# hartikainen/mujoco_mpc

Hardware: AMD Instinct MI355X
Metric: candidate rollouts/s (horizon x samples) (higher is better)
Workload: dtype f64

## Files before the change

mujoco_mpc_amd/csrc/core.h:

```cpp
#pragma once
#include "dmath.h"
#include "model.h"
#include "linalg.h"
#include "philox.h"

#ifdef MJPC_EMU
static thread_local double *g_emu_lds = nullptr;
static thread_local int g_emu_r = 0;
typedef const KParams *KP;
DEV const KParams *kp_generic(KP k) { return k; }
DEV double *lds_base() { return g_emu_lds; }
DEV int cand_index() { return g_emu_r; }
DEV int uniform_i(int v) { return v; }
#else
extern __shared__ __align__(16) double g_lds[];
typedef const __attribute__((address_space(4))) KParams *KP;
DEV const KParams *kp_generic(KP k) {
  unsigned long long v = (unsigned long long)k;
  unsigned lo = __builtin_amdgcn_readfirstlane((unsigned)v), hi = __builtin_amdgcn_readfirstlane((unsigned)(v >> 32));
  KP u = (KP)(((unsigned long long)hi << 32) | lo);
  return (const KParams *)u;
}
DEV double *lds_base() { return g_lds; }
DEV int cand_index() { return (int)blockIdx.x; }
// ... 211 lines not shown
  }
  PFOR(i, M.nmocap) {
    d_copy3(c.mocap_pos + 3 * i, K->mocap + 7 * i);
    d_copy4(c.mocap_quat + 4 * i, K->mocap + 7 * i + 3);
  }
  PFOR(i, nq) { c.qpos[i] = K->state[i]; R.states[i] = K->state[i]; }
  PFOR(i, nv) { c.qvel[i] = K->state[nq + i]; R.states[nq + i] = K->state[nq + i]; c.qacc_ws[i] = 0; }
  if (M.na) PFOR(i, M.na) { C_ACT(c)[i] = K->state[nq + nv + i]; R.states[nq + nv + i] = K->state[nq + nv + i]; C_ACTDOT(c)[i] = 0; }
  PFOR(e, nv * M.nvp) c.qM[e] = 0;
  if (K->L.Linv - K->L.qH >= nv * M.nvp) PFOR(e, nv * M.nvp) c.qH[e] = 0;
#ifndef MJPC_LEAN_LDS
  PFOR(e, M.nhpair + nv) c.hpair[e] = MI(hpair_i)[e] | (MI(hpair_j)[e] << 8);
#endif
#ifndef MJPC_LEAN_LDS
  PFOR(k, 6 * M.nbody) c.xfrc[k] = 0;
#endif
  PFOR(k, nu) c.ctrl[k] = 0;
  if (LANE == 0) {
    R.times[0] = K->time;
    for (int k = 0; k < 3; k++) { c.xpos[k] = 0; c.xipos[k] = 0; c.subtree_linvel[k] = 0; }
    c.xquat[0] = 1; c.xquat[1] = 0; c.xquat[2] = 0; c.xquat[3] = 0;
    for (int k = 0; k < 9; k++) { c.xmat[k] = (k % 4 == 0) ? 1.0 : 0.0; c.ximat[k] = c.xmat[k]; }
    for (int k = 0; k < 6; k++) { c.cvel[k] = 0; c.cfrc[k] = 0; c.cacc[k] = (k >= 3) ? -M.gravity[k - 3] : 0.0; }
    for (int k = 0; k < MISC_INTS; k++) c.misc[k] = 0;
#if defined(MJPC_PROFILE) && !defined(MJPC_EMU)
    for (int q = 0; q < NPROF; q++) c.prof[q] = 0;
    c.prof[NPROF] = (long long)__builtin_amdgcn_s_memtime();
#endif
  }
  c.time = K->time;
  ctx_close(c);
}

template <int NVT>
DEV_NOINLINE void ph_head(KP Kc, int t, int last) {
  Ctx c; ctx_open(c, Kc);
  const KParams *K = c.K;
  const DevModel &M = *c.M;
  Rows R = out_rows(K);
  int nu = M.nu;
  if (!last) {
    PFOR(k, nu) {
      double a = spline_sample(c.knot_times, c.knot_values, K->P, nu, K->interp, c.time, k);
      a = d_clip(a, MD(actuator_ctrlrange)[2 * k], MD(actuator_ctrlrange)[2 * k + 1]);
      c.ctrl[k] = a; R.actions[t * nu + k] = a;
    }
    SYNC();
    if (bad_values(c.qpos, M.nq)) c.warning |= WARN_BADQPOS;
    if (bad_values(c.qvel, M.nv)) c.warning |= WARN_BADQVEL;
    if (c.warning) { if (LANE == 0) c.misc[10] = 1; ctx_close(c); return; }
    if (K->xfrc_std > 0) {
      double rate = exp(-M.timestep / K->xfrc_rate), scale = K->xfrc_std * sqrt(1 - rate * rate);
      unsigned gi = (unsigned)(K->offset + cand_index());
      int n6 = 6 * M.nbody;
      PFOR(i, n6) c.xfrc[i] = rate * c.xfrc[i] + scale * philox_normal(K->seed, K->stream ^ XFRC_STREAM, gi, (unsigned)(t * n6 + i));
    }
  }
  PROF(c, 0);
  kinematics(c); PROF(c, 1);
#if !MJPC_SIDE_COM
  com_pos(c);
#endif
  PROF(c, 2);
  ctx_close(c);
}
DEV_NOINLINE void ph_constraints(KP Kc, int t) {
  Ctx c; ctx_open(c, Kc);
  collision(c); PROF(c, 4);
  int nsingle, n_nc;
#if MJPC_HELPER
#if MJPC_SIDE_COM
  if (!flag_wait(c.misc + HX_COM, t + 1)) c.warning |= WARN_SYNC;
#endif
  if (!flag_wait(c.misc + 24, t + 1)) c.warning |= WARN_SYNC;
  nsingle = uniform_i(c.misc[25]); n_nc = uniform_i(c.misc[26]);
  c.nsingle = nsingle;
  make_contact_rows(c, n_nc); PROF(c, 5);
  make_impedance(c, n_nc, c.nefc, 1); PROF(c, 7);
#else
  make_noncontact_rows(c, &nsingle, &n_nc);
  c.nsingle = nsingle;
  make_contact_rows(c, n_nc); PROF(c, 5);
  make_impedance(c, 0, c.nefc, 1); PROF(c, 7);
#endif
  ctx_close(c);
}
#if MJPC_HELPER
DEV_NOINLINE void ph_noncontact(KP Kc, int t) {
  Ctx c; ctx_open(c, Kc, 1);
  int nsingle, n_nc;
#if MJPC_SIDE_COM
  if (c.M->neq_connect) { if (!flag_wait(c.misc + HX_COM, t + 1)) c.warning |= WARN_SYNC; }
#endif
  make_noncontact_rows(c, &nsingle, &n_nc);
  if (LANE == 0) { c.misc[25] = nsingle; c.misc[26] = n_nc; }
  flag_set(c.misc + 24, t + 1);
// ... 44 lines not shown
DEV_SOLVE_PHASE void ph_solve(KP Kc, int last, int t) {
  Ctx c; ctx_open(c, Kc);
  c.hseq = t * 256;
  solve_constraints<NVT>(c); PROF(c, 8);
#if MJPC_HELPER
  if (MJPC_SOLVER_REG && NVT > 0) { if (c.M->cone == 1) flag_set(c.misc + HX_JOBW, JOBW(++c.hseq, 0, 0)); }
  else {
    if (LANE == 0) c.misc[HX_KIND] = 0;
    flag_set(c.misc + HX_JOB, ++c.hseq);
  }
#endif
  if (!last && !(c.warning & (WARN_CONTACTFULL | WARN_CNSTRFULL)) && bad_values(c.qacc, c.M->nv)) c.warning |= WARN_BADQACC;
  ctx_close(c);
}
template <int NVT>
DEV_NOINLINE void ph_noslip(KP Kc, int last) {
  Ctx c; ctx_open(c, Kc);
  if (!(c.warning & (WARN_CONTACTFULL | WARN_CNSTRFULL | WARN_SYNC | WARN_BADQACC))) {
    noslip_pass<NVT>(c);
    if (!last && bad_values(c.qacc, c.M->nv)) c.warning |= WARN_BADQACC;
  }
  ctx_close(c);
}
#if MJPC_HELPER
template <int NVT>
DEV_NOINLINE void ph_solve_helper(KP Kc, int t) {
  Ctx c; ctx_open(c, Kc, 1);
  int k = WAVE_ID() - 1;
  static_for<0, MJPC_NH>([&](auto Kc_) { constexpr int KK = decltype(Kc_)::value; if (k == KK) solver_helper_loop<NVT, KK>(c, t * 256); });
}
#endif

struct CostOut { double cost; int warning; };
DEV_NOINLINE CostOut ph_residual_cost(KP Kc, int t, int last) {
  Ctx c; ctx_open(c, Kc, 1);
  const KParams *K = c.K;
  const DevModel &M = *c.M;
  const DevTask &T = M.task;
  Rows R = out_rows(K);
  if (last) PFOR(k, M.nu) R.actions[t * M.nu + k] = (K->H > 1) ? c.ctrl[k] : 0.0;
  if (t == 0 && cand_index() == 0 && K->frame) {
    int nb = M.nbody, ns = M.nsite;
    double *f = K->frame;
    PFOR(i, 3 * nb) { f[i] = c.xpos[i]; f[12 * nb + 3 * ns + i] = c.subtree_com[i]; f[15 * nb + 3 * ns + i] = c.subtree_linvel[i]; }
    PFOR(i, 9 * nb) f[3 * nb + i] = c.xmat[i];
    PFOR(i, 3 * ns) f[12 * nb + i] = c.site_xpos[i];
  }
  task_residual(c, c.residual); PROF(c, 9); PROFW(c, 9);
  PFOR(i, R.nr) R.residual[t * R.nr + i] = c.residual[i];
  PFOR(i, T.num_trace) {
    int id = MI(task.trace_objid)[i], ty = MI(task.trace_objtype)[i];
    const double *src = ty == 6 ? c.site_xpos + 3 * id : (ty == 5 ? c.geom_xpos + 3 * id : (ty == 1 ? c.xipos + 3 * id : c.xpos + 3 * id));
    d_copy3(R.trace + t * R.ntr + 3 * i, src);
  }
  CostOut o;
  o.cost = cost_value(c, c.residual);
  if (LANE == 0) R.costs[t] = o.cost;
  o.warning = c.warning;
  PROF(c, 10); PROFW(c, 10);
  ctx_close(c);
  return o;
}

template <int NVT>
DEV void prefactor_body(Ctx &c) {
  const DevModel &M = *c.M;
  {
    int nv = M.nv, nvp = M.nvp;
    double h = M.timestep;
    PFOR(e, nv * nvp) { int i = e / nvp, j = e - i * nvp; c.qL[e] = c.qM[e] + ((i == j) ? h * MD(dof_damping)[i] : 0.0); }
    if (M.nidrv) {
      SYNC();
      if (LANE == 0)
        for (int k = 0; k < M.nidrv; k++) {
          int i = MI(idrv_e)[3 * k], j = MI(idrv_e)[3 * k + 1], a = MI(idrv_e)[3 * k + 2];
          if (a >= 0 && MI(actuator_forcelimited)[a]) {
            double f = c.actuator_force[a];
            if (f <= MD(actuator_forcerange)[2 * a] || f >= MD(actuator_forcerange)[2 * a + 1]) continue;
          }
          double v = h * MD(idrv_c)[k];
          c.qL[i * nvp + j] += v;
          if (i != j) c.qL[j * nvp + i] += v;
        }
      SYNC();
    }
    chol_factor<NVT>(c.qL, c.Linv, c.scr_a, nv, nvp, c.M->tree_ok);
  }
}
template <int NVT>
DEV_NOINLINE void ph_prefactor(KP Kc) {
  Ctx c; ctx_open(c, Kc, 1);
// ... 134 lines not shown
        d_sub3(off, c.xipos + 3 * b, c.subtree_com + 3 * MIH(body_rootid)[b]);
        const double *ci = c.cdof + 6 * i, *cj = c.cdof + 6 * j;
        d_cross(t, ci, off); for (int k = 0; k < 3; k++) { wi[k] = ci[k]; wi[3 + k] = ci[3 + k] + t[k]; }
        d_cross(t, cj, off); for (int k = 0; k < 3; k++) { wj[k] = cj[k]; wj[3 + k] = cj[3 + k] + t[k]; }
        d_mulmattvec3(li, R, wi); d_mulmattvec3(li + 3, R, wi + 3);
        d_mulmattvec3(lj, R, wj); d_mulmattvec3(lj + 3, R, wj + 3);
        for (int k = 0; k < 6; k++) acc += li[k] * dl[k] * lj[k];
      }
      A[i * nvp + j] += h * acc;
    }
    SYNC();
  }
  if (M.int_dense == 2) implicit_rne_columns(c, A, h);
  for (int k = 0; k < nv; k++) {
    SYNC();
    const double piv = A[k * nvp + k];
    PFOR(ii, nv - k - 1) { int i = k + 1 + ii; A[i * nvp + k] = d_div(A[i * nvp + k], piv); }
    SYNC();
    PFOR(e, (nv - k - 1) * (nv - k - 1)) {
      int i = k + 1 + e / (nv - k - 1), j = k + 1 + e % (nv - k - 1);
      A[i * nvp + j] -= A[i * nvp + k] * A[k * nvp + j];
    }
  }
  SYNC();
  double *x = c.Mgrad;
  if (LANE == 0) {
    for (int i = 0; i < nv; i++) { double s = x[i]; for (int j = 0; j < i; j++) s -= A[i * nvp + j] * x[j]; x[i] = s; }
    for (int i = nv - 1; i >= 0; i--) { double s = x[i]; for (int j = i + 1; j < nv; j++) s -= A[i * nvp + j] * x[j]; x[i] = d_div(s, A[i * nvp + i]); }
  }
  SYNC();
}

template <int NVT>
DEV_NOINLINE void ph_integrate(KP Kc, int t) {
  Ctx c; ctx_open(c, Kc);
  const KParams *K = c.K;
  const DevModel &M = *c.M;
  Rows R = out_rows(K);
  int nq = M.nq, nv = M.nv, nvp = M.nvp;
  double h = M.timestep;
  if (M.noslip_iterations <= 0) { PFOR(i, nv) c.qacc_ws[i] = c.qacc[i]; }
  else if (M.any_damping && !M.int_dense) { prefactor_body<NVT>(c); SYNC(); }
  if (M.int_dense) {
    PFOR(i, nv) c.Mgrad[i] = c.qfrc_smooth[i] + c.qfrc_constraint[i];
    SYNC();
    implicit_dense_solve<NVT>(c);
    PFOR(i, nv) c.qvel[i] += h * c.Mgrad[i];
  } else if (M.any_damping) {
    PFOR(i, nv) c.Mgrad[i] = c.qfrc_smooth[i] + c.qfrc_constraint[i];
    chol_solve<NVT>(c.qL, c.Linv, c.Mgrad, nv, nvp, c.M->tree_ok);
    PFOR(i, nv) c.qvel[i] += h * c.Mgrad[i];
  } else {
    PFOR(i, nv) c.qvel[i] += h * c.qacc[i];
  }
  SYNC();
  PFOR(j, M.njnt) {
    int qa = MIH(jnt_qposadr)[j], da = MIH(jnt_dofadr)[j], type = MIH(jnt_type)[j];
    if (type == 0) {
      for (int k = 0; k < 3; k++) c.qpos[qa + k] += h * c.qvel[da + k];
      d_quatintegrate(c.qpos + qa + 3, c.qvel + da + 3, h);
    } else if (type == 1) {
      d_quatintegrate(c.qpos + qa, c.qvel + da, h);
    } else c.qpos[qa] += h * c.qvel[da];
  }
  if (M.na) {
    PFOR(i, M.nu) {
      int dt = MI(actuator_dyntype)[i];
      if (dt) {
        int a = MI(actuator_actadr)[i];
        double act = C_ACT(c)[a], ad = C_ACTDOT(c)[a];
        if (dt == DYN_FILTEREXACT) { double tau = fmax(D_MINVAL, MD(actuator_dynprm)[i]); act += ad * tau * (1 - exp(-h / tau)); }
        else act += h * ad;
        if (MI(actuator_actlimited)[i]) act = d_clip(act, MD(actuator_actrange)[2 * i], MD(actuator_actrange)[2 * i + 1]);
        C_ACT(c)[a] = act;
        R.states[(t + 1) * R.ds + nq + nv + a] = act;
      }
    }
  }
  c.time += h;
  SYNC();
  PFOR(i, nq) R.states[(t + 1) * R.ds + i] = c.qpos[i];
  PFOR(i, nv) R.states[(t + 1) * R.ds + nq + i] = c.qvel[i];
  if (LANE == 0) R.times[t + 1] = c.time;
  PROF(c, 11);
  ctx_close(c);
}

#define CKPT_HEAD 7
DEV_NOINLINE void ph_finish(KP Kc, double total, int failure, int t_fail, double total_before) {
  Ctx c; ctx_open(c, Kc, 1);
  const KParams *K = c.K;
  int r = cand_index(), H = K->H;
  if (K->tier > 0 && K->ckpt) {
    double *ck = K->ckpt + (size_t)r * K->ckpt_stride;
    const DevModel &M = *c.M;
    int resumable = failure && (c.warning & (WARN_CONTACTFULL | WARN_CNSTRFULL)) && !(c.warning & ~(WARN_CONTACTFULL | WARN_CNSTRFULL)) && !(K->xfrc_std > 0);
    if (LANE == 0) {
      ck[0] = resumable ? 1.0 : 0.0; ck[1] = (double)t_fail; ck[2] = c.time; ck[3] = total_before;
      ck[4] = (double)c.misc[5]; ck[5] = (double)c.misc[6]; ck[6] = (double)c.misc[7];
    }
    if (resumable) {
      PFOR(i, M.nq) ck[CKPT_HEAD + i] = c.qpos[i];
      PFOR(i, M.nv) { ck[CKPT_HEAD + M.nq + i] = c.qvel[i]; ck[CKPT_HEAD + M.nq + M.nv + i] = c.qacc_ws[i]; }
      if (M.na) PFOR(i, M.na) ck[CKPT_HEAD + M.nq + 2 * M.nv + i] = C_ACT(c)[i];
    }
  }
  if (LANE == 0) {
    K->returns[r] = failure ? 1.0e6 : total / (H > 1 ? H : 1);
    K->failure[r] = failure ? (c.warning ? c.warning : 1) : 0;
#if defined(MJPC_PROFILE) && !defined(MJPC_EMU)
    if (K->prof) for (int q = 0; q < NPROF; q++) K->prof[(size_t)r * NPROF + q] = c.prof[q];
#endif
    if (K->diag) { K->diag[4 * r] = c.misc[5]; K->diag[4 * r + 1] = c.misc[6]; K->diag[4 * r + 2] = c.misc[7]; K->diag[4 * r + 3] = c.warning; }
  }
}

DEV_NOINLINE void ph_resume(KP Kc) {
// ... 5 lines not shown
  PFOR(i, M.nv) { c.qvel[i] = ck[CKPT_HEAD + M.nq + i]; c.qacc_ws[i] = ck[CKPT_HEAD + M.nq + M.nv + i]; }
  if (M.na) PFOR(i, M.na) C_ACT(c)[i] = ck[CKPT_HEAD + M.nq + 2 * M.nv + i];
  if (LANE == 0) { c.misc[5] = (int)ck[4]; c.misc[6] = (int)ck[5]; c.misc[7] = (int)ck[6]; }
  c.time = ck[2];
  ctx_close(c);
}

template <int NVT>
DEV void rollout(KP Kc) {
  int H = Kc->H;
  const bool r0 = ROLE0, r1 = ROLE1;
  if (r0) ph_init(Kc);
  XBAR();
  const int *misc = (const int *)(lds_base() + Kc->L.ints) + Kc->L.i_misc;
  double total = 0, total_before = 0;
  int failure = 0, t0 = 0, t_fail = 0;
  if (Kc->retry && Kc->ckpt) {
    const double *ck = Kc->ckpt + (size_t)cand_index() * Kc->ckpt_stride;
    if (ck[0] != 0.0) {
      t0 = (int)ck[1]; total = ck[3];
      if (r0) ph_resume(Kc);
      XBAR();
    }
  }
#if defined(MJPC_PROFILE) && !defined(MJPC_EMU)
  long long *rprof = (long long *)(lds_base() + Kc->L.prof);
#define RPROF(i) do { if (LANE == 0 && WAVE_ID() == MJPC_PROFILE_WAVE) PROF_STAMP(rprof, i); } while (0)
#else
#define RPROF(i) ((void)0)
#endif
  for (int t = t0; t < H; t++) {
    int last = (t == H - 1);
    t_fail = t; total_before = total;
    if (r0) ph_head<NVT>(Kc, t, last);
    XBAR(); RPROF(2);
    if (uniform_i(misc[10])) { failure = 1; break; }
    if (r0) ph_constraints(Kc, t);
    if (r1) ph_smooth<NVT>(Kc, t);
#if MJPC_HELPER
    if (ROLEH && WAVE_ID() == 1) ph_inertia<NVT>(Kc, t);
    if (ROLEH && WAVE_ID() == MJPC_WAVES - 2) ph_noncontact(Kc, t);
#endif
    XBAR(); RPROF(3);
    if (r0) { ph_solve<NVT>(Kc, last, t); if (Kc->M.noslip_iterations > 0) ph_noslip<NVT>(Kc, last); }
#if MJPC_HELPER
    if (ROLEH) ph_solve_helper<NVT>(Kc, t);
#endif
    if (r1) {
      CostOut o = ph_residual_cost(Kc, t, last); total += o.cost;
      if (!last) ph_prefactor<NVT>(Kc);
#if MJPC_HELPER
      ph_side_worker<NVT>(Kc, t);
#endif
    }
    XBAR(); RPROF(6);
    if (uniform_i(misc[3]) | uniform_i(misc[11])) { failure = 1; break; }
    if (r0 && !last) ph_integrate<NVT>(Kc, t);
  }
  XBAR();
  if (r1) ph_finish(Kc, total, failure, t_fail, total_before);
}
```

mujoco_mpc_amd/csrc/linalg.h:

```cpp
#pragma once
#include <type_traits>
#include "dmath.h"
#include "model.h"

struct Ctx;

#ifndef MJPC_EMU
DEV double readlane_d(double v, int lane) {
  int lo = __builtin_amdgcn_readlane(__double2loint(v), lane);
  int hi = __builtin_amdgcn_readlane(__double2hiint(v), lane);
  return __hiloint2double(hi, lo);
}
#endif

DEV void chol_factor_lds(double *A, double *Linv, double *tmp, int n, int nvp) {
  for (int j = 0; j < n; j++) {
    SYNC();
    PFOR(ii, n - j) {
      int i = j + ii;
      double s = A[i * nvp + j];
#pragma unroll 4
      for (int k = 0; k < j; k++) s -= A[i * nvp + k] * A[j * nvp + k];
      tmp[i] = s;
    }
    SYNC();
    double t = tmp[j];
    if (t < D_MINVAL) t = D_MINVAL;
    double dj = sqrt(t), inv = 1.0 / dj;
    PFOR(ii, n - j) {
      int i = j + ii;
      A[i * nvp + j] = (i == j) ? dj : tmp[i] * inv;
    }
    if (LANE == 0) Linv[j] = inv;
  }
  SYNC();
}
DEV void chol_solve_lds(const double *L, const double *Linv, double *x, int n, int nvp) {
  for (int i = 0; i < n; i++) {
    SYNC();
    double xi = x[i] * Linv[i];
    SYNC();
    PFOR(kk, n - i - 1) { int k = i + 1 + kk; x[k] -= L[k * nvp + i] * xi; }
    if (LANE == 0) x[i] = xi;
  }
  for (int i = n - 1; i >= 0; i--) {
    SYNC();
    double xi = x[i] * Linv[i];
    SYNC();
    PFOR(k, i) x[k] -= L[i * nvp + k] * xi;
    if (LANE == 0) x[i] = xi;
  }
  SYNC();
}

#ifndef MJPC_EMU
template <int N>
struct LDLRegs { double lo[N], up[N], rinv; };
struct LDLExtra { const double *x[3]; int n; const double *row; };

template <int I, int E, class F>
DEV void static_for(F &&f) {
  if constexpr (I < E) { f(std::integral_constant<int, I>{}); static_for<I + 1, E>(f); }
}
template <int N>
DEV void ldl_load_row(const double *A, int nvp, const LDLExtra *ex, double *a, double &dg) {
  const int i = LANE;
  const bool act = i < N;
  if (ex && ex->row) {
    double d0 = 1.0;
    static_for<0, N>([&](auto jc) { constexpr int j = decltype(jc)::value; a[j] = act ? ex->row[j] : 0.0; d0 = (j == i) ? ex->row[j] : d0; });
    dg = act ? d0 : 1.0;
  } else {
    static_for<0, N>([&](auto jc) { constexpr int j = decltype(jc)::value; a[j] = act ? A[(j <= i) ? i * nvp + j : j * nvp + i] : 0.0; });
    dg = act ? A[i * nvp + i] : 1.0;
  }
  if (ex && ex->n > 0) {
    const int nx = ex->n;
    double t[3][N], td[3];
#pragma unroll
    for (int w = 0; w < 3; w++) {
      const double *X = ex->x[w < nx ? w : 0];
      static_for<0, N>([&](auto jc) { constexpr int j = decltype(jc)::value; t[w][j] = X[(j <= i && act) ? i * nvp + j : (act ? j * nvp + i : 0)]; });
      td[w] = X[act ? i * nvp + i : 0];
      if (w + 1 >= nx) break;
    }
    __builtin_amdgcn_sched_barrier(0);
#pragma unroll
    for (int w = 0; w < 3; w++) {
      if (w >= nx) break;
      static_for<0, N>([&](auto jc) { constexpr int j = decltype(jc)::value; a[j] += act ? t[w][j] : 0.0; });
      dg += act ? td[w] : 0.0;
    }
  }
}
template <int N>
DEV void ldl_factor_regs(const double *A, int nvp, LDLRegs<N> &f, const LDLExtra *ex = nullptr) {
  static_assert(N >= 1 && N <= 64, "one matrix row per lane");
  const int i = LANE;
  const bool act = i < N;
  double a[N];
  double dg;
  ldl_load_row<N>(A, nvp, ex, a, dg);
  static_for<1, N>([&](auto kc) {
// ... 192 lines not shown
```

mujoco_mpc_amd/csrc/solver_reg.h:

```cpp
#pragma once
#ifndef MJPC_EMU
#ifndef LS_PREDICT
#define LS_PREDICT 1
#endif

template <int NVT> struct HLay {
  static constexpr int G0 = 64 / NVT;
  static constexpr int G = G0 < 1 ? 1 : (G0 > NVT ? NVT : G0);
  static constexpr int CB = (NVT + G - 1) / G;
};
DEV int readlane_i(int v, int lane) { return __builtin_amdgcn_readlane(v, lane); }
#define LSR_STRIDE 7
#define LSC_STRIDE 17
#define LS_ROWREC(c) ((c).efc_JA + 64)
#define LS_CONREC(c) ((c).efc_JA + 64 + (c).M->nefcmax * LSR_STRIDE)

template <int NVT>
DEV void hblock_add_rows(const Ctx &c, double *h, unsigned long long mask, int rbase, double wlane, int hi, int j0) {
  constexpr int nvp = NVP_OF(NVT), CB = HLay<NVT>::CB;
  while (mask) {
    int b0 = (int)__builtin_ctzll(mask); mask &= mask - 1;
    int b1 = b0; double sel1 = 0.0;
    if (mask) { b1 = (int)__builtin_ctzll(mask); mask &= mask - 1; sel1 = 1.0; }
    double w0 = readlane_d(wlane, b0), w1 = readlane_d(wlane, b1) * sel1;
// ... 112 lines not shown
#if defined(MJPC_PROFILE) && !defined(MJPC_EMU)
    if (MJPC_PROFILE_WAVE != 0 && WAVE_ID() == MJPC_PROFILE_WAVE) { int na_ = __builtin_popcountll(__builtin_amdgcn_ballot_w64(active)); if (LANE == 0) { c.prof[23] += na_; c.prof[22] += (it0 == p0 * NLANE); } }
#endif
    if constexpr (DIMT > 3) {
#pragma unroll
      for (int k = 3; k < DIMT; k++) { const bool in = k < dim; P[k] = in ? P[k] : 0.0; Q[k] = in ? Q[k] : 0.0; T[k] = in ? T[k] : 0.0; ji[k] = in ? ji[k] : 0.0; }
    }
    double pi = P[0] * ji[0], qi = Q[1] * ji[1];
#pragma unroll
    for (int k = 1; k < DIMT; k++) { pi += P[k] * ji[k]; if (k > 1) qi += Q[k] * ji[k]; }
    double t[DIMT];
    t[0] = P[0] * pi + Q[0] * ji[0];
#pragma unroll
    for (int k = 1; k < DIMT; k++) t[k] = P[k] * pi - Q[k] * qi + (T[k] * T[k]) * ji[k];
    double *prow = part + i * nvp;
    PROFW(c, 16);
    for (int b = 0; __builtin_amdgcn_ballot_w64(active && b <= a) != 0; b += 2) {
      const bool on0 = active && b <= a, on1 = active && b + 1 <= a;
      const int j0 = dofs[on0 ? b : 0], j1 = dofs[on1 ? b + 1 : 0];
      double x0[DIMT], x1[DIMT];
#pragma unroll
      for (int k = 0; k < DIMT; k++) { x0[k] = Jr[(DIMT <= 3 || k < dim ? k : 0) * nvp + j0]; x1[k] = Jr[(DIMT <= 3 || k < dim ? k : 0) * nvp + j1]; }
      __builtin_amdgcn_sched_barrier(0);
      double v0 = t[0] * x0[0], v1 = t[0] * x1[0];
#pragma unroll
      for (int k = 1; k < DIMT; k++) { v0 += t[k] * x0[k]; v1 += t[k] * x1[k]; }
      if (on0) __builtin_amdgcn_ds_atomic_fadd_f64((__attribute__((address_space(3))) double *)(prow + j0), v0);
      if (on1) __builtin_amdgcn_ds_atomic_fadd_f64((__attribute__((address_space(3))) double *)(prow + j1), v1);
    }
  }
}

#if MJPC_HELPER
DEV int jobw_load(const Ctx &c) { return __builtin_amdgcn_readfirstlane(__hip_atomic_load(c.misc + HX_JOBW, __ATOMIC_RELAXED, __HIP_MEMORY_SCOPE_WORKGROUP)); }
template <int NVT>
DEV int job_post(Ctx &c, int kind, int &side_in) {
  if (c.M->cone != 1) return 0;
  const int seq = ++c.hseq;
  if (MJPC_SIDE_JOB > 0 && !side_in && (seq & 255) >= MJPC_SIDE_JOB) {
    const int base = seq & ~255;
    int ok = 0;
    for (int n = 0; n < (1 << 21); n++) {
      int from = __builtin_amdgcn_readfirstlane(__hip_atomic_load(c.misc + HX_SIDEFROM, __ATOMIC_RELAXED, __HIP_MEMORY_SCOPE_WORKGROUP));
      if (from > base) { ok = 1; break; }
    }
    if (!ok) c.warning |= WARN_SYNC;
    side_in = 1;
  }
  const int np = MJPC_NH + (side_in ? 1 : 0);
  flag_set(c.misc + HX_JOBW, JOBW(seq, np, kind));
  return np;
}
DEV void job_wait(Ctx &c, int np) {
  const int seq = c.hseq;
  for (int k = 0; k < np; k++) if (!flag_wait(c.misc + HX_WDONE + k, seq)) c.warning |= WARN_SYNC;
}
template <int NVT, int DIMT>
DEV void worker_job(Ctx &c, int W, int np, int seq) {
  constexpr int nvp = NVP_OF(NVT);
  PROFW(c, 12);
  double *part = CONE_PARTIAL(c, W);
  PFOR(e, NVT * nvp) part[e] = 0;
  PROFW(c, 15);
  cone_rows<NVT, DIMT>(c, part, W, np);
  PROFW(c, 13);
  flag_set(c.misc + HX_WDONE + W, seq);
  PROFW(c, 14);
}
template <int NVT, int DIMT>
DEV void worker_loop_d(Ctx &c, int W, int last) {
  if (W != 0 && c.nefc > 0 && !flag_wait(c.misc + HX_LSREC, (last >> 8) + 1)) return;
  for (;;) {
    int word = 0, ok = 0;
    for (int n = 0; n < (1 << 21); n++) { word = jobw_load(c); if ((word >> 4) > last) { ok = 1; break; } }
    __builtin_amdgcn_fence(__ATOMIC_ACQUIRE, "workgroup");
    if (!ok) return;
    const int kind = word & 3, np = (word >> 2) & 3;
    if (kind == 0) return;
    last = word >> 4;
    if (W < np) worker_job<NVT, DIMT>(c, W, np, last);
  }
}
template <int NVT>
DEV void worker_loop(Ctx &c, int W, int last) {
  if (c.M->cone != 1) return;
  if (c.M->maxdim <= 3) worker_loop_d<NVT, 3>(c, W, last); else worker_loop_d<NVT, 6>(c, W, last);
}
template <int NVT>
DEV void side_worker(Ctx &c, int t) {
  if (c.M->cone != 1 || MJPC_SIDE_JOB <= 0) return;
  const int base = t * 256;
  int word = jobw_load(c);
  int last = base;
  if ((word >> 4) > base) {
    if ((word & 3) == 0) return;
    last = word >> 4;
  }
  if (LANE == 0) __hip_atomic_store(c.misc + HX_SIDEFROM, last + 1, __ATOMIC_RELAXED, __HIP_MEMORY_SCOPE_WORKGROUP);
  worker_loop<NVT>(c, MJPC_NH, last);
}
#endif

template <int NVT, int DIMT>
DEV void newton_assemble(Ctx &c, const double *hq, int hi, int hg, int j0, bool hact) {
  constexpr int nvp = NVP_OF(NVT), CB = HLay<NVT>::CB;
  double a[CB];
  const double dg = c.sgl[NVT + hi] + c.sgl[3 * NVT + hi];
#pragma unroll
  for (int q = 0; q < CB; q++) a[q] = hq[q] + ((j0 + q == hi) ? dg : 0.0);
#if !MJPC_HELPER
  if (c.M->cone == 1) {
    double *part = CONE_PARTIAL(c, 0);
    PFOR(e, NVT * nvp) part[e] = 0;
    cone_rows<NVT, DIMT>(c, part, 0, 1);
    SYNC();
#pragma unroll
    for (int q = 0; q < CB; q++) a[q] += (hact && j0 + q <= hi) ? part[hi * nvp + j0 + q] : 0.0;
  }
#endif
  if (hact) {
#pragma unroll
    for (int q = 0; q < CB; q++) if (j0 + q < NVT) c.qH[hi * nvp + j0 + q] = a[q];
  }
  SYNC();
}
template <int NVT>
DEV void newton_direction_np(Ctx &c, int np) {
  if (np > 0) {
    LDLExtra ex;
    ex.row = nullptr;
    ex.n = np;
#pragma unroll
    for (int w = 0; w < 3; w++) ex.x[w] = CONE_PARTIAL(c, w < np ? w : 0);
    newton_direction_sum<NVT>(c, ex);
  } else newton_direction<NVT>(c);
}

template <int NVT>
DEV void newton_direction_rows(Ctx &c, const double *hq, int hi, bool hact, int np) {
  if constexpr (HLay<NVT>::G != 1) return;
  double row[NVT];
  const double dg = c.sgl[NVT + hi] + c.sgl[3 * NVT + hi];
#pragma unroll
  for (int q = 0; q < NVT; q++) row[q] = hact ? hq[q] + ((q == hi) ? dg : 0.0) : 0.0;
  LDLExtra ex;
  ex.row = row;
  ex.n = np;
#pragma unroll
  for (int w = 0; w < 3; w++) ex.x[w] = CONE_PARTIAL(c, w < np ? w : 0);
  chol_factor_solve_reg<NVT>(c.qH, c.Mgrad, NVP_OF(NVT), c.M->tree_ok && !c.cross, &ex);
  PROF(c, 17);
}

template <int DIMT>
struct LSReg {
  double lo[LS_RPL], hi[LS_RPL], hD[LS_RPL], F[LS_RPL], X[LS_RPL], V[LS_RPL], DV[LS_RPL], DVV[LS_RPL], rJ[LS_RPL];
  int rinfo[LS_RPL];
  double N0[LS_CPL], NV[LS_CPL], t0[LS_CPL], t1[LS_CPL], t2[LS_CPL], c0[LS_CPL], c1[LS_CPL], c2[LS_CPL], mu[LS_CPL], Dm[LS_CPL];
  int on[LS_CPL], cdim[LS_CPL], crow[LS_CPL], cwasq[LS_CPL];
  int nslot, ncslot;
};

template <int NVT>
DEV void ls_records_build(Ctx &c) {
  constexpr int nvp = NVP_OF(NVT);
  const int nefc = c.nefc, ncon = c.ncon, ns = c.nsingle, nfr = c.M->nfric;
  double *rrec = LS_ROWREC(c), *crec = LS_CONREC(c);
  PFOR(r, nefc) {
    int type = c.efc_type[r], dof = c.efc_dof[r];
    double D = c.efc_D[r], f = c.efc_floss[r], Rf = c.efc_R[r] * f;
    int single = r < ns;
    double rj = single ? (r < nfr ? 1.0 : c.efc_J[r * nvp + dof]) : 0.0;
    int quad = type != CNSTR_CONTACT_ELLIPTIC;
    int fric = quad && type <= CNSTR_FRICTION_TENDON;
    double *o = rrec + r * LSR_STRIDE;
    o[0] = fric ? -Rf : (quad ? -1e300 : -1.0); o[1] = fric ? Rf : (quad ? 0.0 : 1.0);
    o[2] = quad ? 0.5 * D : 0.0; o[3] = fric ? f : 0.0; o[4] = rj;
    ((int *)(o + 5))[0] = quad | (fric << 1) | ((quad && single) << 2) | ((single ? dof : 0) << 8);
    o[6] = D;
  }
  int nc_lane = 0;
  PFOR(ci, ncon) {
    int dim = c.con_i[ci * CONI_STRIDE], i = c.con_i[ci * CONI_STRIDE + 3];
    const double *cc = c.contact + ci * c.M->con_stride;
// ... 256 lines not shown
#else
  cost_sm = solver_eval<NVT>(c, c.qacc_smooth, 0);
  double cost_ws = solver_eval<NVT>(c, c.qacc_ws, &gauss);
#endif
  if (cost_ws > cost_sm) {
    PFOR(i, nv) c.qacc[i] = c.qacc_smooth[i];
    SYNC();
    cost = solver_eval<NVT>(c, c.qacc, &gauss);
  } else {
    PFOR(i, nv) c.qacc[i] = c.qacc_ws[i];
    SYNC();
    cost = cost_ws;
  }
  PROF(c, 12);
  int np = 0, side_in = 0;
  int ncone = 0;
  if (c.M->cone == 1) {
    const int ci = LANE < c.ncon ? LANE : 0;
    const int dim = c.con_i[ci * CONI_STRIDE], r0c = c.con_i[ci * CONI_STRIDE + 3];
    const int stc = c.efc_state[r0c];
    ncone = __builtin_popcountll(__builtin_amdgcn_ballot_w64(LANE < c.ncon && dim > 1 && stc == STATE_CONE));
  }
#if MJPC_HELPER
  if (ncone) np = job_post<NVT>(c, 1, side_in);
#else
  ls_records_build<NVT>(c);
#endif
  double hq[CB];
  hblock_init<NVT>(c, hq, hi, j0);
  PROF(c, 15);
  newton_grad_reg<NVT>(c, hi, hg, hact);
  PROF(c, 9);
  if constexpr (!ROWS) { newton_assemble<NVT, DIMT>(c, hq, hi, hg, j0, hact); PROF(c, 19); }
#if MJPC_HELPER
  if (np) { job_wait(c, np); PROF(c, 16); }
#endif
  if constexpr (!ROWS) newton_direction_np<NVT>(c, np); else newton_direction_rows<NVT>(c, hq, hi, hact, np);
  PFOR(i, nv) c.search[i] = -c.Mgrad[i];
  SYNC();
  const double scale = 1.0 / (M.meaninertia * (nv > 1 ? nv : 1));
  for (int iter = 0; iter < M.iterations; iter++) {
    PROF(c, 13);
    double p_sn = 0, p_q1 = 0, p_q2 = 0, p_gs = 0;
    mat_rows_times<NVT>(c, c.search, c.Mv, c.efc_jv);
    PFOR(i, nv) {
      double si = c.search[i];
      p_sn += si * si; p_q1 += si * (c.Ma[i] - c.qfrc_smooth[i]); p_q2 += 0.5 * si * c.Mv[i]; p_gs += c.grad[i] * si;
    }
    SYNC();
    wave_sum4(p_sn, p_q1, p_q2, p_gs);
    const double snorm = sqrt(p_sn), q1 = p_q1, q2 = p_q2, gs = p_gs;
    PROF(c, 20);
    if (snorm < D_MINVAL || gs >= 0) break;
    const double gtol = M.tolerance * M.ls_tolerance * snorm / scale;
    LSReg<DIMT> d;
#if MJPC_HELPER
    if (iter == 0 && !flag_wait(c.misc + HX_LSREC, c.hseq / 256 + 1)) c.warning |= WARN_SYNC;
#endif
    ls_load_reg<NVT, DIMT>(c, d);
    PROF(c, 21);
    double lo = 0, hi_a = -1, a = 1.0;
    double best_a = 0, best_cost = cost, dxold = a, dx = a;
    LSPoint p; p.cost = cost; p.d1 = gs; p.d2 = -gs;
    int moved = 0;
    const double pred_tol = 1e-3 * M.tolerance / scale;
    for (int it = 0; it < M.ls_iterations; it++) {
      p = ls_eval_reg<DIMT>(d, gauss, q1, q2, a);
#if defined(MJPC_PROFILE) && !defined(MJPC_EMU)
      if (LANE == 0) c.prof[23] += 1;
#endif
// ... 21 lines not shown
      a = an;
    }
    PROF(c, 22);
    const double alpha = moved ? a : best_a;
    PROF(c, 14);
    if (alpha == 0) break;
    unsigned long long chg_mask[LS_RPL]; double chg_w[LS_RPL];
    const double ccost = ls_commit<NVT, DIMT>(c, d, alpha, chg_mask, chg_w, &ncone);
    PFOR(i, nv) { c.qacc[i] += alpha * c.search[i]; c.Ma[i] += alpha * c.Mv[i]; }
    SYNC();
    gauss = gauss + alpha * q1 + alpha * alpha * q2;
    const double oldcost = cost;
    cost = gauss + ccost;
    PROF(c, 12);
    const double improvement = scale * (oldcost - cost);
    const int stop = improvement < M.tolerance || (c.warning & WARN_SYNC) != 0;
#if MJPC_HELPER
    np = (stop || !ncone) ? 0 : job_post<NVT>(c, 1, side_in);
#endif
    if (!stop) {
#pragma unroll
      for (int k = 0; k < LS_RPL; k++) { if (k >= d.nslot) break; hblock_add_rows<NVT>(c, hq, chg_mask[k], NLANE * k, chg_w[k], hi, j0); }
    }
    PROF(c, 15);
    newton_grad_reg<NVT>(c, hi, hg, hact);
    PROF(c, 9);
    c.solver_iter++;
    double pg = 0;
    PFOR(i, nv) pg += c.grad[i] * c.grad[i];
    const double gradient = scale * sqrt(wave_sum(pg));
    const int done = stop || gradient < M.tolerance;
    if constexpr (!ROWS) { if (!done) { newton_assemble<NVT, DIMT>(c, hq, hi, hg, j0, hact); PROF(c, 19); } }
#if MJPC_HELPER
    if (np) { job_wait(c, np); PROF(c, 16); }
#endif
    if (done) break;
    if constexpr (!ROWS) newton_direction_np<NVT>(c, np); else newton_direction_rows<NVT>(c, hq, hi, hact, np);
    PFOR(i, nv) c.search[i] = -c.Mgrad[i];
    SYNC();
  }
  if (LANE == 0) { c.misc[5] += c.solver_iter; if (c.ncon > c.misc[6]) c.misc[6] = c.ncon; if (c.nefc > c.misc[7]) c.misc[7] = c.nefc; }
  PFOR(i, nv) c.qfrc_constraint[i] = (c.Ma[i] - c.qfrc_smooth[i]) - c.grad[i];
  SYNC();
}

template <int NVT>
DEV void solve_constraints_reg(Ctx &c) {
  if (c.M->maxdim <= 3) solve_constraints_reg_d<NVT, 3>(c); else solve_constraints_reg_d<NVT, 6>(c);
}
#endif
```

Baseline: 25220.

## Fuse integrate with next head, defer row stores, preload cone data, prefetch Hessian row

Merges the integrate phase with the next step's head into one call and moves the state/action row stores into the residual-cost phase on the other role. The next step's control is computed early, at the end of the cost phase. Helper workers preload their cone Jacobian columns once per solve into registers, and the main wave loads its Hessian row before waiting on helper jobs, so load latency overlaps the wait. The aim is fewer phase calls and barriers and hidden memory latency, at the cost of more register pressure and trickier handling of rows on the failure path.

```diff
diff --git a/mujoco_mpc_amd/csrc/core.h b/mujoco_mpc_amd/csrc/core.h
--- a/mujoco_mpc_amd/csrc/core.h
+++ b/mujoco_mpc_amd/csrc/core.h
@@ -267,23 +267,45 @@
   ctx_close(c);
 }
 
-template <int NVT>
-DEV_NOINLINE void ph_head(KP Kc, int t, int last) {
-  Ctx c; ctx_open(c, Kc);
+DEV void policy_to_ctrl(Ctx &c, double time) {
   const KParams *K = c.K;
-  const DevModel &M = *c.M;
-  Rows R = out_rows(K);
-  int nu = M.nu;
+  const int nu = c.M->nu;
+  PFOR(k, nu) {
+    double a = spline_sample(c.knot_times, c.knot_values, K->P, nu, K->interp, time, k);
+    c.ctrl[k] = d_clip(a, MD(actuator_ctrlrange)[2 * k], MD(actuator_ctrlrange)[2 * k + 1]);
+  }
+}
+DEV void store_step_rows(Ctx &c, const Rows &R, int t, int last) {
+  const DevModel &M = *c.M;
+  const int nq = M.nq, nv = M.nv, nu = M.nu;
+  PFOR(i, nq) R.states[t * R.ds + i] = c.qpos[i];
+  PFOR(i, nv) R.states[t * R.ds + nq + i] = c.qvel[i];
+  if (M.na) PFOR(i, M.na) R.states[t * R.ds + nq + nv + i] = C_ACT(c)[i];
+  if (LANE == 0) R.times[t] = c.time;
+  if (!last) PFOR(k, nu) R.actions[t * nu + k] = c.ctrl[k];
+}
+DEV_NOINLINE void ph_rows(KP Kc, int t, int last) {
+  Ctx c; ctx_open(c, Kc, 1);
+  Rows R = out_rows(c.K);
+  store_step_rows(c, R, t, last);
+  ctx_close(c);
+}
+
+template <int NVT>
+DEV int head_body(Ctx &c, int t, int last, int first) {
+  const KParams *K = c.K;
+  const DevModel &M = *c.M;
   if (!last) {
-    PFOR(k, nu) {
-      double a = spline_sample(c.knot_times, c.knot_values, K->P, nu, K->interp, c.time, k);
-      a = d_clip(a, MD(actuator_ctrlrange)[2 * k], MD(actuator_ctrlrange)[2 * k + 1]);
-      c.ctrl[k] = a; R.actions[t * nu + k] = a;
+    if (first) {
+      Rows R = out_rows(K);
+      policy_to_ctrl(c, c.time);
+      SYNC();
+      PFOR(k, M.nu) R.actions[t * M.nu + k] = c.ctrl[k];
     }
     SYNC();
     if (bad_values(c.qpos, M.nq)) c.warning |= WARN_BADQPOS;
     if (bad_values(c.qvel, M.nv)) c.warning |= WARN_BADQVEL;
-    if (c.warning) { if (LANE == 0) c.misc[10] = 1; ctx_close(c); return; }
+    if (c.warning) { if (LANE == 0) c.misc[10] = 1; return 0; }
     if (K->xfrc_std > 0) {
       double rate = exp(-M.timestep / K->xfrc_rate), scale = K->xfrc_std * sqrt(1 - rate * rate);
       unsigned gi = (unsigned)(K->offset + cand_index());
@@ -297,6 +319,12 @@
   com_pos(c);
 #endif
   PROF(c, 2);
+  return 1;
+}
+template <int NVT>
+DEV_NOINLINE void ph_head(KP Kc, int t, int last) {
+  Ctx c; ctx_open(c, Kc);
+  head_body<NVT>(c, t, last, 1);
   ctx_close(c);
 }
 DEV_NOINLINE void ph_constraints(KP Kc, int t) {
@@ -407,12 +435,13 @@
 #endif
 
 struct CostOut { double cost; int warning; };
-DEV_NOINLINE CostOut ph_residual_cost(KP Kc, int t, int last) {
+DEV_NOINLINE CostOut ph_residual_cost(KP Kc, int t, int last, int rows) {
   Ctx c; ctx_open(c, Kc, 1);
   const KParams *K = c.K;
   const DevModel &M = *c.M;
   const DevTask &T = M.task;
   Rows R = out_rows(K);
+  if (rows) store_step_rows(c, R, t, last);
   if (last) PFOR(k, M.nu) R.actions[t * M.nu + k] = (K->H > 1) ? c.ctrl[k] : 0.0;
   if (t == 0 && cand_index() == 0 && K->frame) {
     int nb = M.nbody, ns = M.nsite;
@@ -432,6 +461,7 @@
   o.cost = cost_value(c, c.residual);
   if (LANE == 0) R.costs[t] = o.cost;
   o.warning = c.warning;
+  if (!last && t + 1 < K->H - 1) { SYNC(); policy_to_ctrl(c, c.time + M.timestep); }
   PROF(c, 10); PROFW(c, 10);
   ctx_close(c);
   return o;
@@ -632,12 +662,9 @@
 }
 
 template <int NVT>
-DEV_NOINLINE void ph_integrate(KP Kc, int t) {
-  Ctx c; ctx_open(c, Kc);
-  const KParams *K = c.K;
-  const DevModel &M = *c.M;
-  Rows R = out_rows(K);
-  int nq = M.nq, nv = M.nv, nvp = M.nvp;
+DEV void integrate_body(Ctx &c) {
+  const DevModel &M = *c.M;
+  int nv = M.nv, nvp = M.nvp;
   double h = M.timestep;
   if (M.noslip_iterations <= 0) { PFOR(i, nv) c.qacc_ws[i] = c.qacc[i]; }
   else if (M.any_damping && !M.int_dense) { prefactor_body<NVT>(c); SYNC(); }
@@ -673,16 +700,18 @@
         else act += h * ad;
         if (MI(actuator_actlimited)[i]) act = d_clip(act, MD(actuator_actrange)[2 * i], MD(actuator_actrange)[2 * i + 1]);
         C_ACT(c)[a] = act;
-        R.states[(t + 1) * R.ds + nq + nv + a] = act;
       }
     }
   }
   c.time += h;
   SYNC();
-  PFOR(i, nq) R.states[(t + 1) * R.ds + i] = c.qpos[i];
-  PFOR(i, nv) R.states[(t + 1) * R.ds + nq + i] = c.qvel[i];
-  if (LANE == 0) R.times[t + 1] = c.time;
   PROF(c, 11);
+}
+template <int NVT>
+DEV_NOINLINE void ph_integrate_head(KP Kc, int t, int last_next) {
+  Ctx c; ctx_open(c, Kc);
+  integrate_body<NVT>(c);
+  head_body<NVT>(c, t + 1, last_next, 0);
   ctx_close(c);
 }
 
@@ -754,9 +783,9 @@
   for (int t = t0; t < H; t++) {
     int last = (t == H - 1);
     t_fail = t; total_before = total;
-    if (r0) ph_head<NVT>(Kc, t, last);
+    if (r0 && t == t0) ph_head<NVT>(Kc, t, last);
     XBAR(); RPROF(2);
-    if (uniform_i(misc[10])) { failure = 1; break; }
+    if (uniform_i(misc[10])) { if (r1 && t > t0) ph_rows(Kc, t, last); failure = 1; break; }
     if (r0) ph_constraints(Kc, t);
     if (r1) ph_smooth<NVT>(Kc, t);
 #if MJPC_HELPER
@@ -769,7 +798,7 @@
     if (ROLEH) ph_solve_helper<NVT>(Kc, t);
 #endif
     if (r1) {
-      CostOut o = ph_residual_cost(Kc, t, last); total += o.cost;
+      CostOut o = ph_residual_cost(Kc, t, last, t > t0); total += o.cost;
       if (!last) ph_prefactor<NVT>(Kc);
 #if MJPC_HELPER
       ph_side_worker<NVT>(Kc, t);
@@ -777,7 +806,7 @@
     }
     XBAR(); RPROF(6);
     if (uniform_i(misc[3]) | uniform_i(misc[11])) { failure = 1; break; }
-    if (r0 && !last) ph_integrate<NVT>(Kc, t);
+    if (r0 && !last) ph_integrate_head<NVT>(Kc, t, t + 1 == H - 1);
   }
   XBAR();
   if (r1) ph_finish(Kc, total, failure, t_fail, total_before);
diff --git a/mujoco_mpc_amd/csrc/linalg.h b/mujoco_mpc_amd/csrc/linalg.h
--- a/mujoco_mpc_amd/csrc/linalg.h
+++ b/mujoco_mpc_amd/csrc/linalg.h
@@ -56,7 +56,7 @@
 #ifndef MJPC_EMU
 template <int N>
 struct LDLRegs { double lo[N], up[N], rinv; };
-struct LDLExtra { const double *x[3]; int n; const double *row; };
+struct LDLExtra { const double *x[3]; int n; const double *row; const double *diag = nullptr; };
 
 template <int I, int E, class F>
 DEV void static_for(F &&f) {
@@ -68,7 +68,11 @@
   const bool act = i < N;
   if (ex && ex->row) {
     double d0 = 1.0;
-    static_for<0, N>([&](auto jc) { constexpr int j = decltype(jc)::value; a[j] = act ? ex->row[j] : 0.0; d0 = (j == i) ? ex->row[j] : d0; });
+    if (ex->diag) {
+      static_for<0, N>([&](auto jc) { constexpr int j = decltype(jc)::value; a[j] = act ? ex->row[j] : 0.0; });
+      d0 = *ex->diag;
+    } else
+      static_for<0, N>([&](auto jc) { constexpr int j = decltype(jc)::value; a[j] = act ? ex->row[j] : 0.0; d0 = (j == i) ? ex->row[j] : d0; });
     dg = act ? d0 : 1.0;
   } else {
     static_for<0, N>([&](auto jc) { constexpr int j = decltype(jc)::value; a[j] = act ? A[(j <= i) ? i * nvp + j : j * nvp + i] : 0.0; });
diff --git a/mujoco_mpc_amd/csrc/solver_reg.h b/mujoco_mpc_amd/csrc/solver_reg.h
--- a/mujoco_mpc_amd/csrc/solver_reg.h
+++ b/mujoco_mpc_amd/csrc/solver_reg.h
@@ -168,6 +168,83 @@
 }
 
 #if MJPC_HELPER
+#define CONE_PRE_COLS 12
+template <int DIMT>
+struct ConePre {
+  int ok;
+  int valid, a, r0, ioff;
+  const double *cf;
+  double ji[DIMT];
+  int j[CONE_PRE_COLS];
+  double x[CONE_PRE_COLS][DIMT];
+};
+template <int NVT, int DIMT>
+DEV void cone_preload(const Ctx &c, int W, ConePre<DIMT> &p) {
+  constexpr int nvp = NVP_OF(NVT);
+  p.ok = 0;
+  if constexpr (DIMT > 3) return;
+  if (c.nefc <= 0 || W >= MJPC_NH) return;
+  const int nitems = uniform_i(c.misc[HX_NITEMS]), stride = c.M->con_stride;
+  if (nitems > MJPC_NH * NLANE) return;
+  const unsigned short *items = CONE_ITEMS(c);
+  const double *crec = LS_CONREC(c);
+  const int it = W * NLANE + LANE;
+  const bool valid = it < nitems;
+  const int item = items[valid ? it : 0];
+  const int ci = item & 255, a = item >> 8;
+  if (__builtin_amdgcn_ballot_w64(valid && a >= CONE_PRE_COLS) != 0) return;
+  const int info = ((const int *)(crec + ci * LSC_STRIDE + 14))[0];
+  const int r0 = info >> 16;
+  const unsigned char *dofs = CONE_DOFS(c) + ci * NVT;
+  const int i = dofs[a];
+  const double *Jr = c.efc_J + r0 * nvp;
+  p.valid = valid; p.a = a; p.r0 = r0; p.ioff = i * nvp;
+  p.cf = c.contact + ci * stride + CON_H;
+#pragma unroll
+  for (int k = 0; k < DIMT; k++) p.ji[k] = Jr[k * nvp + i];
+#pragma unroll
+  for (int b = 0; b < CONE_PRE_COLS; b++) {
+    const int jb = dofs[(valid && b <= a) ? b : 0];
+    p.j[b] = jb;
+#pragma unroll
+    for (int k = 0; k < DIMT; k++) p.x[b][k] = Jr[k * nvp + jb];
+  }
+  p.ok = 1;
+}
+template <int NVT, int DIMT>
+DEV void cone_rows_pre(const Ctx &c, const ConePre<DIMT> &p, double *part) {
+  const int st = c.efc_state[p.r0];
+  const double *cf = p.cf;
+  double P[DIMT], Q[DIMT], T[DIMT], ji[DIMT];
+#pragma unroll
+  for (int k = 0; k < DIMT; k++) { P[k] = cf[k]; Q[k] = cf[6 + k]; T[k] = cf[12 + k]; ji[k] = p.ji[k]; }
+  __builtin_amdgcn_sched_barrier(0);
+  const int a = p.a;
+  const bool active = p.valid && st == STATE_CONE;
+#if defined(MJPC_PROFILE) && !defined(MJPC_EMU)
+  if (MJPC_PROFILE_WAVE != 0 && WAVE_ID() == MJPC_PROFILE_WAVE) { int na_ = __builtin_popcountll(__builtin_amdgcn_ballot_w64(active)); if (LANE == 0) { c.prof[23] += na_; c.prof[22] += 1; } }
+#endif
+  double pi = P[0] * ji[0], qi = Q[1] * ji[1];
+#pragma unroll
+  for (int k = 1; k < DIMT; k++) { pi += P[k] * ji[k]; if (k > 1) qi += Q[k] * ji[k]; }
+  double t[DIMT];
+  t[0] = P[0] * pi + Q[0] * ji[0];
+#pragma unroll
+  for (int k = 1; k < DIMT; k++) t[k] = P[k] * pi - Q[k] * qi + (T[k] * T[k]) * ji[k];
+  double *prow = part + p.ioff;
+  PROFW(c, 16);
+#pragma unroll
+  for (int b = 0; b < CONE_PRE_COLS; b += 2) {
+    if (__builtin_amdgcn_ballot_w64(active && b <= a) == 0) break;
+    const bool on0 = active && b <= a, on1 = active && b + 1 <= a;
+    double v0 = t[0] * p.x[b][0], v1 = t[0] * p.x[b + 1][0];
+#pragma unroll
+    for (int k = 1; k < DIMT; k++) { v0 += t[k] * p.x[b][k]; v1 += t[k] * p.x[b + 1][k]; }
+    if (on0) __builtin_amdgcn_ds_atomic_fadd_f64((__attribute__((address_space(3))) double *)(prow + p.j[b]), v0);
+    if (on1) __builtin_amdgcn_ds_atomic_fadd_f64((__attribute__((address_space(3))) double *)(prow + p.j[b + 1]), v1);
+  }
+}
+
 DEV int jobw_load(const Ctx &c) { return __builtin_amdgcn_readfirstlane(__hip_atomic_load(c.misc + HX_JOBW, __ATOMIC_RELAXED, __HIP_MEMORY_SCOPE_WORKGROUP)); }
 template <int NVT>
 DEV int job_post(Ctx &c, int kind, int &side_in) {
@@ -192,13 +269,14 @@
   for (int k = 0; k < np; k++) if (!flag_wait(c.misc + HX_WDONE + k, seq)) c.warning |= WARN_SYNC;
 }
 template <int NVT, int DIMT>
-DEV void worker_job(Ctx &c, int W, int np, int seq) {
+DEV void worker_job(Ctx &c, int W, int np, int seq, const ConePre<DIMT> &pre) {
   constexpr int nvp = NVP_OF(NVT);
   PROFW(c, 12);
   double *part = CONE_PARTIAL(c, W);
   PFOR(e, NVT * nvp) part[e] = 0;
   PROFW(c, 15);
-  cone_rows<NVT, DIMT>(c, part, W, np);
+  if (pre.ok && np >= MJPC_NH) cone_rows_pre<NVT, DIMT>(c, pre, part);
+  else cone_rows<NVT, DIMT>(c, part, W, np);
   PROFW(c, 13);
   flag_set(c.misc + HX_WDONE + W, seq);
   PROFW(c, 14);
@@ -206,6 +284,9 @@
 template <int NVT, int DIMT>
 DEV void worker_loop_d(Ctx &c, int W, int last) {
   if (W != 0 && c.nefc > 0 && !flag_wait(c.misc + HX_LSREC, (last >> 8) + 1)) return;
+  ConePre<DIMT> pre;
+  cone_preload<NVT, DIMT>(c, W, pre);
+  PROFW(c, 18);
   for (;;) {
     int word = 0, ok = 0;
     for (int n = 0; n < (1 << 21); n++) { word = jobw_load(c); if ((word >> 4) > last) { ok = 1; break; } }
@@ -214,7 +295,7 @@
     const int kind = word & 3, np = (word >> 2) & 3;
     if (kind == 0) return;
     last = word >> 4;
-    if (W < np) worker_job<NVT, DIMT>(c, W, np, last);
+    if (W < np) worker_job<NVT, DIMT>(c, W, np, last, pre);
   }
 }
 template <int NVT>
@@ -261,10 +342,19 @@
   SYNC();
 }
 template <int NVT>
-DEV void newton_direction_np(Ctx &c, int np) {
+DEV void newton_row_load(const Ctx &c, double *row, double &dg) {
+  constexpr int nvp = NVP_OF(NVT);
+  const int i = LANE;
+  const bool act = i < NVT;
+  static_for<0, NVT>([&](auto jc) { constexpr int j = decltype(jc)::value; row[j] = act ? c.qH[(j <= i) ? i * nvp + j : j * nvp + i] : 0.0; });
+  dg = act ? c.qH[i * nvp + i] : 1.0;
+}
+template <int NVT>
+DEV void newton_direction_np(Ctx &c, int np, const double *row = nullptr, const double *dg = nullptr) {
   if (np > 0) {
     LDLExtra ex;
-    ex.row = nullptr;
+    ex.row = row;
+    ex.diag = dg;
     ex.n = np;
 #pragma unroll
     for (int w = 0; w < 3; w++) ex.x[w] = CONE_PARTIAL(c, w < np ? w : 0);
@@ -286,6 +376,29 @@
   for (int w = 0; w < 3; w++) ex.x[w] = CONE_PARTIAL(c, w < np ? w : 0);
   chol_factor_solve_reg<NVT>(c.qH, c.Mgrad, NVP_OF(NVT), c.M->tree_ok && !c.cross, &ex);
   PROF(c, 17);
+}
+
+template <int NVT, bool ROWS>
+DEV void solve_direction(Ctx &c, const double *hq, int hi, bool hact, int np) {
+  if constexpr (ROWS) {
+#if MJPC_HELPER
+    if (np) { job_wait(c, np); PROF(c, 16); }
+#endif
+    newton_direction_rows<NVT>(c, hq, hi, hact, np);
+  } else {
+#if MJPC_HELPER
+    if (HLay<NVT>::G > 1 && np) {
+      double row[NVT], dg;
+      newton_row_load<NVT>(c, row, dg);
+      __builtin_amdgcn_sched_barrier(0);
+      job_wait(c, np); PROF(c, 16);
+      newton_direction_np<NVT>(c, np, row, &dg);
+      return;
+    }
+    if (np) { job_wait(c, np); PROF(c, 16); }
+#endif
+    newton_direction_np<NVT>(c, np);
+  }
 }
 
 template <int DIMT>
@@ -608,10 +721,7 @@
   newton_grad_reg<NVT>(c, hi, hg, hact);
   PROF(c, 9);
   if constexpr (!ROWS) { newton_assemble<NVT, DIMT>(c, hq, hi, hg, j0, hact); PROF(c, 19); }
-#if MJPC_HELPER
-  if (np) { job_wait(c, np); PROF(c, 16); }
-#endif
-  if constexpr (!ROWS) newton_direction_np<NVT>(c, np); else newton_direction_rows<NVT>(c, hq, hi, hact, np);
+  solve_direction<NVT, ROWS>(c, hq, hi, hact, np);
   PFOR(i, nv) c.search[i] = -c.Mgrad[i];
   SYNC();
   const double scale = 1.0 / (M.meaninertia * (nv > 1 ? nv : 1));
@@ -699,10 +809,11 @@
     const int done = stop || gradient < M.tolerance;
     if constexpr (!ROWS) { if (!done) { newton_assemble<NVT, DIMT>(c, hq, hi, hg, j0, hact); PROF(c, 19); } }
 #if MJPC_HELPER
-    if (np) { job_wait(c, np); PROF(c, 16); }
-#endif
+    if (done) { if (np) { job_wait(c, np); PROF(c, 16); } break; }
+#else
     if (done) break;
-    if constexpr (!ROWS) newton_direction_np<NVT>(c, np); else newton_direction_rows<NVT>(c, hq, hi, hact, np);
+#endif
+    solve_direction<NVT, ROWS>(c, hq, hi, hact, np);
     PFOR(i, nv) c.search[i] = -c.Mgrad[i];
     SYNC();
   }
```

Result: no change. 25060 (-0.6%).
